# CMU-SAFARI/RawAlign

Measured on AMD Instinct MI355X. Metric: DTW GCUPS, higher is better.
Workload: dtype f32; 1 GPU; ecoli_k12_4.6Mb_r9.4_sparse_banded0.10; reads_per_gpu=16384, genome_bp=4600000, border_constraint=sparse, fill_method=banded=0.10, batches_in_flight=4

## Files before the change

rawalign_amd/csrc/rawdtw_runs.hip:

```cpp

#include "rawdtw_dp.h"

namespace rawdtw {

namespace {

constexpr int kT = 256;

__device__ __forceinline__ int d_slanted_radius(uint32_t n, uint32_t m, int r0)
{
    const uint32_t N = n > m ? n : m, M = n > m ? m : n;
    const uint32_t x = (N - M) * (uint32_t)r0 + N - 1u;
    uint32_t q;
    if (N < (1u << 11) && (uint32_t)r0 < (1u << 11)) {
        q = (uint32_t)((float)x * __builtin_amdgcn_rcpf((float)N));
        const int r = (int)x - (int)(q * N);
        q = r < 0 ? q - 1u : (r >= (int)N ? q + 1u : q);
    } else q = x / N;
    return r0 + (int)q;
}

__device__ uint32_t d_banded_cells(uint32_t n, uint32_t m, int R)
{
    const uint32_t N = n > m ? n : m, M = n > m ? m : n;
    const int P = R + ((R % 2 == 0) ? 1 : 0), S = R + ((R % 2 == 1) ? 1 : 0);
    uint32_t cells = 1;
    int row = 0;
    uint32_t rem = 0;
    for (uint32_t col = 1; col < N; col++) {
        rem += M;
        const bool adv = rem >= N;
        if (adv) { rem -= N; row++; }
        for (int pass = adv ? 0 : 1; pass < 2; pass++) {
            const int len = pass == 0 ? S : P;
            const int si = pass == 0 ? (int)col + S / 2 - 1 : (int)col + P / 2;
            const int sj = pass == 0 ? row - S / 2 : row - P / 2;
            int lo = 0, hi = len;
            lo = max(lo, si - (int)N + 1);
            lo = max(lo, -sj);
            hi = min(hi, si + 1);
            hi = min(hi, (int)M - sj);
            if (hi > lo) cells += (uint32_t)(hi - lo);
        }
    }
    return cells;
}

struct Part {
    uint32_t n, m;
    int R;
    bool asc;
    bool tile;
};

__device__ __forceinline__ Part classify(const StreamArgs &a, const rawdtw_anchor_t s, const rawdtw_anchor_t e)
{
    Part p;
    p.asc = e.target_position >= s.target_position && e.query_position >= s.query_position;
    p.m = e.target_position - s.target_position + 1;
    p.n = e.query_position - s.query_position + 1;
    int r0 = (int)((float)p.n * a.frac);
    r0 = r0 > 1 ? r0 : 1;
    const uint32_t N = p.n > p.m ? p.n : p.m, dr = (N - (p.n > p.m ? p.m : p.n)) * (uint32_t)r0;
    p.R = r0 + (dr > 0u ? 1 : 0) + (dr > N ? 1 : 0);
    p.tile = p.asc && p.n < 0x7fffffffu && p.m < 0x7fffffffu && N <= a.lane_max_n && r0 <= a.lane_max_radius &&
             dr <= (uint32_t)(a.lane_max_radius - r0) * N;
    return p;
}

__device__ __forceinline__ uint64_t find_chain(const uint64_t *__restrict__ anchor_off, uint64_t n_chains, uint64_t x, int lane)
{
    uint64_t lo = 0, hi = n_chains;
    while (hi - lo > 1) {
        const uint64_t step = (hi - lo + 63) / 64;
        const uint64_t p = lo + (uint64_t)lane * step;
        const bool le = p < hi && anchor_off[p] <= x;
        const int cnt = __popcll(__ballot(le));
        const uint64_t nlo = lo + (uint64_t)(cnt - 1) * step;
        hi = min(hi, nlo + step);
        lo = nlo;
    }
    return lo;
}

__device__ __forceinline__ void wave_lds_sync()
{
    __builtin_amdgcn_fence(__ATOMIC_RELEASE, "wavefront");
    __builtin_amdgcn_wave_barrier();
    __builtin_amdgcn_fence(__ATOMIC_ACQUIRE, "wavefront");
}

__device__ __forceinline__ uint32_t wave_scan_incl(uint32_t x)
{
    x += (uint32_t)__builtin_amdgcn_update_dpp(0, (int)x, 0x111, 0xf, 0xf, false);
    x += (uint32_t)__builtin_amdgcn_update_dpp(0, (int)x, 0x112, 0xf, 0xf, false);
    x += (uint32_t)__builtin_amdgcn_update_dpp(0, (int)x, 0x114, 0xf, 0xf, false);
    x += (uint32_t)__builtin_amdgcn_update_dpp(0, (int)x, 0x118, 0xf, 0xf, false);
    x += (uint32_t)__builtin_amdgcn_update_dpp(0, (int)x, 0x142, 0xa, 0xf, false);
    x += (uint32_t)__builtin_amdgcn_update_dpp(0, (int)x, 0x143, 0xc, 0xf, false);
    return x;
}

struct StepMap { uint32_t set, q, t; };
__device__ __forceinline__ StepMap compose(const StepMap later, const StepMap earlier)
{
    if (later.set) return later;
    return StepMap{earlier.set, earlier.set ? earlier.q - later.q : earlier.q + later.q, earlier.set ? earlier.t - later.t : earlier.t + later.t};
}
#define RAWDTW_DPP_MAP(m, ctrl, rowmask)                                                                                      \
    StepMap{(uint32_t)__builtin_amdgcn_update_dpp(0, (int)(m).set, ctrl, rowmask, 0xf, false),                                  \
            (uint32_t)__builtin_amdgcn_update_dpp(0, (int)(m).q, ctrl, rowmask, 0xf, false),                                    \
            (uint32_t)__builtin_amdgcn_update_dpp(0, (int)(m).t, ctrl, rowmask, 0xf, false)}
__device__ __forceinline__ StepMap wave_scan_maps(StepMap m)
{
    m = compose(m, RAWDTW_DPP_MAP(m, 0x111, 0xf));
    m = compose(m, RAWDTW_DPP_MAP(m, 0x112, 0xf));
    m = compose(m, RAWDTW_DPP_MAP(m, 0x114, 0xf));
    m = compose(m, RAWDTW_DPP_MAP(m, 0x118, 0xf));
    m = compose(m, RAWDTW_DPP_MAP(m, 0x142, 0xa));
    m = compose(m, RAWDTW_DPP_MAP(m, 0x143, 0xc));
    return m;
}

__device__ __forceinline__ bool mask_bit(const uint32_t *mask, uint32_t p) { return (mask[p >> 5] >> (p & 31u)) & 1u; }

template <int NT>
__device__ __forceinline__ bool mark_chain_starts(const StreamArgs &a, uint64_t c0, uint64_t base, uint32_t at, uint32_t *mask)
{
    bool ok = true;
    for (uint64_t c = c0 + threadIdx.x;; c += NT) {
        uint64_t s = ~0ull;
        if (c <= a.n_chains) {
            s = a.anchor_off[c];
            if (s >= base && s <= base + at) atomicOr(&mask[(uint32_t)(s - base) >> 5], 1u << ((uint32_t)(s - base) & 31u));
            if (c < a.n_chains && s < base + at && a.anchor_off[c + 1] == s) ok = false;
        }
        if (!__syncthreads_or(threadIdx.x == NT - 1 && c < a.n_chains && s < base + at)) break;
    }
    return ok;
}

}

__device__ __forceinline__ void chain_desc_body(const StreamArgs &a, ChainDesc *__restrict__ chains, const uint64_t c)
{
    if (c >= a.n_chains) return;
    const uint64_t a0 = a.anchor_off[c], a1 = a.anchor_off[c + 1];
    ChainDesc d;
    d.job_first = a1 >= 2 ? a1 - 2 : 0;
    d.n_jobs = a1 > a0 ? (uint32_t)(a1 - a0 - 1) : 0u;
    d.descending = 1; d.span = 0; d.num_aligned = 0;
    if (a1 > a0) {
        const rawdtw_anchor_t first = a.anchors[a1 - 1], last = a.anchors[a0];
        d.span = last.query_position - first.query_position + 1;
        d.num_aligned = (last.query_position - first.query_position) + d.n_jobs;
        if (d.n_jobs && ((uint64_t)a.read_base[c] + last.query_position + 1ull > a.n_ev || a.ref_base[c] + last.target_position + 1ull > a.n_ref))
            atomicMin(&a.cnt[kCntBad], (unsigned long long)a0);
    } else atomicAdd(&a.cnt[kCntUnsupported], 1ull);
    chains[c] = d;
}

template <int NT>
__device__ __forceinline__ void fold_order_body(const uint64_t n_chains, const uint64_t *__restrict__ anchor_off, uint32_t *__restrict__ order)
{
    constexpr uint32_t kBins = 1024, kB = kBins / NT;
    constexpr uint32_t kC = 4;
    __shared__ uint32_t hist[kBins];
    __shared__ uint32_t wsum[NT / 64];
    const uint32_t tid = threadIdx.x, lane = tid & 63u, wv = tid >> 6;
    auto bucket = [](uint64_t anchors) { return 1023u - (uint32_t)min<uint64_t>(anchors ? anchors - 1 : 0, 1023ull); };
    auto keys = [&](uint64_t c0, uint32_t (&b)[kC]) {
        uint64_t lo[kC], hi[kC];
#pragma unroll
        for (uint32_t q = 0; q < kC; q++) {
            const uint64_t c = min(c0 + (uint64_t)q * NT, n_chains - 1);
            lo[q] = anchor_off[c]; hi[q] = anchor_off[c + 1];
        }
#pragma unroll
        for (uint32_t q = 0; q < kC; q++) b[q] = bucket(hi[q] - lo[q]);
    };
    for (uint32_t i = tid; i < kBins; i += NT) hist[i] = 0;
    __syncthreads();
    for (uint64_t c0 = tid; c0 < n_chains; c0 += (uint64_t)NT * kC) {
        uint32_t b[kC];
        keys(c0, b);
#pragma unroll
        for (uint32_t q = 0; q < kC; q++)
            if (c0 + (uint64_t)q * NT < n_chains) atomicAdd(&hist[b[q]], 1u);
    }
    __syncthreads();
    uint32_t v[kB], mine = 0;
#pragma unroll
    for (uint32_t q = 0; q < kB; q++) { v[q] = hist[tid * kB + q]; mine += v[q]; }
    uint32_t incl = mine;
#pragma unroll
    for (int d = 1; d < 64; d <<= 1) {
        const uint32_t o = (uint32_t)__shfl_up((int)incl, d);
        if (lane >= (uint32_t)d) incl += o;
    }
    if (lane == 63) wsum[wv] = incl;
    __syncthreads();
    uint32_t at = incl - mine;
    for (uint32_t w = 0; w < wv; w++) at += wsum[w];
#pragma unroll
    for (uint32_t q = 0; q < kB; q++) { hist[tid * kB + q] = at; at += v[q]; }
    __syncthreads();
    for (uint64_t c0 = tid; c0 < n_chains; c0 += (uint64_t)NT * kC) {
        uint32_t b[kC];
        keys(c0, b);
#pragma unroll
        for (uint32_t q = 0; q < kC; q++)
            if (c0 + (uint64_t)q * NT < n_chains) order[atomicAdd(&hist[b[q]], 1u)] = (uint32_t)(c0 + (uint64_t)q * NT);
    }
}

struct RunTab {
    uint32_t lo[2][kStreamMaxSeg];
    uint32_t end[2][kStreamMaxSeg];
    int32_t D[2][kStreamMaxSeg];
    long long src[2][kStreamMaxSeg];
};

constexpr uint32_t kScanUnit = 8192, kScanKI = 8;
constexpr uint32_t kScanT = 512, kScanTC = 1024;
static_assert(kScanUnit == RAWDTW_COMPACT_STRIDE, "the compact hand-over is decoded unit by unit");
template <bool COMPACT>
__device__ __forceinline__ void scan_unit_body(const StreamArgs &a, const uint32_t unit)
{
    constexpr int NT = COMPACT ? (int)kScanTC : (int)kScanT, KI = (int)kScanKI;
    constexpr uint32_t AT = kScanUnit, kWords = AT / 32 + 1, kHalf = (uint32_t)NT * KI, kHalves = AT / kHalf;
    static_assert(kHalves * kHalf == AT && (!COMPACT || kHalves == 1), "a unit in whole passes; the compact form in one");
    __shared__ uint32_t s_mask[kWords], s_pre[kWords];
    __shared__ uint32_t s_ocnt, s_obase, s_cls[kStreamClasses];
    __shared__ unsigned long long s_stats[3];
    __shared__ uint64_t s_c0;
    __shared__ uint32_t s_todo;
    constexpr uint32_t kOList = 2048;
    __shared__ uint32_t s_olist[kOList];
    const int tid = threadIdx.x, lane = tid & 63;
    const uint64_t base = (uint64_t)unit * AT;
    for (uint32_t w = tid; w < kWords; w += NT) s_mask[w] = 0;
    if (tid == 0) { s_ocnt = 0; s_todo = 0; }
    if (tid < 3) s_stats[tid] = 0;
    if (tid < (int)kStreamClasses) s_cls[tid] = 0;
    const uint64_t i0 = base + (uint64_t)tid * KI;
    rawdtw_anchor_t an[KI + 1];
    uint4 steps8 = make_uint4(0u, 0u, 0u, 0u);
    if (COMPACT) { if (i0 < a.n_anchors) steps8 = *reinterpret_cast<const uint4 *>(a.steps + i0); }
    else {
#pragma unroll
        for (int k = 0; k <= KI; k++) an[k] = i0 + k < a.n_anchors ? a.anchors[i0 + k] : rawdtw_anchor_t{0, 0};
    }
    const rawdtw_anchor_t *const anchors_rd = COMPACT ? a.anchors_w : a.anchors;
    if (tid < 64) {
        const uint64_t c = find_chain(a.anchor_off, a.n_chains, base, lane);
        if (tid == 0) s_c0 = c;
    }
    __syncthreads();
    const uint64_t c0 = s_c0;
    if (!mark_chain_starts<NT>(a, c0, base, AT, s_mask)) atomicAdd(&a.cnt[kCntUnsupported], 1ull);
    {
        static_assert(kWords <= (uint32_t)NT, "one mask word a thread");
        __shared__ uint32_t s_wsum[NT / 64];
        const uint32_t pc = (uint32_t)tid < kWords ? __popc(s_mask[tid]) : 0u;
        uint32_t incl = pc;
#pragma unroll
        for (int d = 1; d < 64; d <<= 1) {
            const uint32_t o = (uint32_t)__shfl_up((int)incl, d);
            if (lane >= d) incl += o;
        }
        if (lane == 63) s_wsum[tid >> 6] = incl;
        __syncthreads();
        uint32_t pre = 0;
        for (int w = 0; w < (tid >> 6); w++) pre += s_wsum[w];
        if ((uint32_t)tid < kWords) s_pre[tid] = pre + incl - pc;
    }
    __syncthreads();
    auto chain_at = [&](uint32_t p) {
        return c0 + (s_pre[p >> 5] + __popc(s_mask[p >> 5] & (0xffffffffu >> (31u - (p & 31u)))) - (s_mask[0] & 1u));
    };
    if (COMPACT) {
        static_assert(KI == 8, "eight 2-byte steps a thread");
        __shared__ StepMap s_wagg[NT / 64];
        __shared__ uint2 s_first[NT];
        const uint32_t sv[8] = {steps8.x & 0xffffu, steps8.x >> 16, steps8.y & 0xffffu, steps8.y >> 16,
                                steps8.z & 0xffffu, steps8.z >> 16, steps8.w & 0xffffu, steps8.w >> 16};
        StepMap part[KI];
        StepMap run{0u, 0u, 0u};
#pragma unroll
        for (int k = 0; k < KI; k++) {
            const uint32_t p = (uint32_t)tid * KI + k;
            const uint64_t i = base + p;
            StepMap m{0u, 0u, 0u};
            if (i < a.n_anchors) {
                if (mask_bit(s_mask, p)) { const rawdtw_anchor_t h = a.heads[chain_at(p)]; m = StepMap{1u, h.query_position, h.target_position}; }
                else if (p == 0) { const rawdtw_anchor_t h = a.unit_abs[unit]; m = StepMap{1u, h.query_position, h.target_position}; }
                else if (sv[k] == 0xffffu) {
                    uint64_t lo = 0, hi = a.n_wide;
                    while (lo < hi) { const uint64_t mid = (lo + hi) >> 1; if (a.wide[mid].index < (uint32_t)i) lo = mid + 1; else hi = mid; }
                    if (lo < a.n_wide && a.wide[lo].index == (uint32_t)i) m = StepMap{0u, a.wide[lo].query_step, a.wide[lo].target_step};
                    else atomicMin(&a.cnt[kCntBad], (unsigned long long)i);
                } else m = StepMap{0u, sv[k] & 0xffu, sv[k] >> 8};
            }
            run = compose(m, run);
            part[k] = run;
        }
        const StepMap incl = wave_scan_maps(run);
        if (lane == 63) s_wagg[tid >> 6] = incl;
        __syncthreads();
        StepMap pre = RAWDTW_DPP_MAP(incl, 0x138, 0xf);
        {
            StepMap wpre{0u, 0u, 0u};
            for (int w = 0; w < (tid >> 6); w++) wpre = compose(s_wagg[w], wpre);
            pre = compose(pre, wpre);
        }
#pragma unroll
        for (int k = 0; k < KI; k++) {
            const StepMap f = compose(part[k], pre);
            an[k] = rawdtw_anchor_t{f.t, f.q};
            if (i0 + k < a.n_anchors) a.anchors_w[i0 + k] = an[k];
        }
        s_first[tid] = make_uint2(an[0].target_position, an[0].query_position);
        __syncthreads();
        if (tid + 1 < NT) { const uint2 x = s_first[tid + 1]; an[KI] = rawdtw_anchor_t{x.x, x.y}; }
        else an[KI] = base + AT < a.n_anchors ? a.unit_abs[unit + 1] : rawdtw_anchor_t{0, 0};
    }

    uint32_t my_tiles = 0, my_bytes = 0;
    unsigned long long my_obytes = 0;
    uint32_t o_rec[kHalves][KI];
#pragma unroll
    for (uint32_t h = 0; h < kHalves; h++) {
    const uint64_t ih = i0 + (uint64_t)h * kHalf;
    if (h) {
#pragma unroll
        for (int k = 0; k <= KI; k++) an[k] = ih + k < a.n_anchors ? a.anchors[ih + k] : rawdtw_anchor_t{0, 0};
    }
    uint32_t half_tiles = 0;
#pragma unroll
    for (int k = 0; k < KI; k++) {
        o_rec[h][k] = 0xffffffffu;
        const uint32_t p = h * kHalf + (uint32_t)tid * KI + k;
        const uint64_t i = base + p;
        if (i >= a.n_anchors || mask_bit(s_mask, p + 1)) continue;
        const Part pt = classify(a, an[k + 1], an[k]);
        if (!pt.asc || pt.n >= 0x7fffffffu || pt.m >= 0x7fffffffu) { atomicMin(&a.cnt[kCntBad], (unsigned long long)i); continue; }
        if (pt.tile) { my_tiles++; half_tiles++; my_bytes += 4u * (pt.n + pt.m) + 36u; continue; }
        int r0 = (int)((float)pt.n * a.frac);
        r0 = r0 > 1 ? r0 : 1;
        const int R = d_slanted_radius(pt.n, pt.m, r0);
        const uint32_t N = pt.n > pt.m ? pt.n : pt.m, K = (uint32_t)R + 1u;
        uint32_t cls;
        if (R >= 1 && R <= a.side_lane_radius && N <= a.lane_max_n) cls = kClsL0 + side_lane_bucket(N);
        else if (K <= 8) cls = kClsM0 + side_lane_bucket(N);
        else if (K <= 16) cls = kClsG16;
        else if (K <= 256) cls = N >= 1024 ? kClsW0 : N >= 256 ? kClsW0 + 1 : N >= 64 ? kClsW0 + 2 : kClsW0 + 3;
        else { atomicAdd(&a.cnt[kCntUnsupported], 1ull); continue; }
        my_obytes += 4ull * ((unsigned long long)pt.n + pt.m) + 36ull;
        {
            const uint32_t slot = atomicAdd(&s_ocnt, 1u);
            if (slot < kOList) s_olist[slot] = p | (cls << 13) | ((uint32_t)R << 18);
            else o_rec[h][k] = slot | (cls << 16) | ((uint32_t)R << 21);
        }
        atomicAdd(&s_cls[cls], 1u);
    }
    {
        const unsigned long long any_tile = __ballot(half_tiles != 0u);
        if (lane == 0 && any_tile) atomicOr(&s_todo, 1u << ((h * kHalf + (uint32_t)tid * KI) / a.tile_anchors));
    }
    }
    {
        unsigned long long packed = (unsigned long long)my_tiles | ((unsigned long long)my_bytes << 20);
        for (int off = 32; off > 0; off >>= 1) packed += __shfl_down(packed, off);
        if (lane == 0) { atomicAdd(&s_stats[0], packed & 0xfffffull); atomicAdd(&s_stats[1], packed >> 20); }
        if (my_obytes) atomicAdd(&s_stats[2], my_obytes);
    }
    __syncthreads();
    if (tid == 0 && s_ocnt) s_obase = (uint32_t)atomicAdd(&a.cnt[kCntOthers], (unsigned long long)s_ocnt);
    if (tid == 0 && s_todo) {
        const uint32_t tiles_per_unit = AT / a.tile_anchors, todo = s_todo;
        uint64_t at = atomicAdd(&a.cnt[kCntTodo], (unsigned long long)__popc(todo));
        for (uint32_t t = 0; t < tiles_per_unit; t++)
            if ((todo >> t) & 1u) a.tlist[at++] = make_uint2(unit * tiles_per_unit + t, (uint32_t)chain_at(t * a.tile_anchors));
    }
    if (tid < 3) a.tile_stats[3ull * unit + tid] = s_stats[tid];
    if (tid < (int)kStreamClasses && s_cls[tid]) atomicAdd(&a.cnt[kCntCls0 + tid], (unsigned long long)s_cls[tid]);
    __syncthreads();
    auto side_record = [&](const uint32_t p, const uint32_t cls, const uint32_t R, const uint64_t q) {
        if (q >= a.others_cap) return;
        const uint64_t c = chain_at(p);
        const rawdtw_anchor_t e = anchors_rd[base + p];
        const rawdtw_anchor_t s = (COMPACT && p + 1u == AT) ? a.unit_abs[unit + 1] : anchors_rd[base + p + 1];
        DevJob d;
        d.ref_off = a.ref_base[c] + s.target_position;
        d.read_off = a.read_base[c] + s.query_position;
        d.n = e.query_position - s.query_position + 1;
        d.m = e.target_position - s.target_position + 1;
        d.R = (int32_t)R;
        d.flags = mask_bit(s_mask, p) ? 0u : kFlagExcludeLast;
        d.aux = (uint32_t)(base + p);
        a.omix[q] = d; a.ocls[q] = (uint8_t)cls;
    };
    for (uint32_t t = (uint32_t)tid; t < min(s_ocnt, kOList); t += NT) {
        const uint32_t w = s_olist[t];
        side_record(w & 0x1fffu, (w >> 13) & 0x1fu, w >> 18, (uint64_t)s_obase + t);
    }
    if (s_ocnt > kOList) {
        const uint64_t obase = s_obase;
#pragma unroll
        for (uint32_t h = 0; h < kHalves; h++)
#pragma unroll
            for (int k = 0; k < KI; k++) {
                if (o_rec[h][k] == 0xffffffffu) continue;
                side_record(h * kHalf + (uint32_t)tid * KI + k, (o_rec[h][k] >> 16) & 0x1fu, o_rec[h][k] >> 21, obase + (o_rec[h][k] & 0xffffu));
            }
    }
}

__device__ __forceinline__ void chain_desc_carry(const StreamArgs &a, ChainDesc *__restrict__ chains, const uint64_t c)
{
    if (c >= a.n_chains) return;
    const uint64_t f0 = a.full_off[c], f1 = a.full_off[c + 1], r0 = a.anchor_off[c], r1 = a.anchor_off[c + 1];
    const rawdtw_carry_t rec = a.carry[c];
    ChainDesc d;
    d.job_first = f1 >= 2 ? f1 - 2 : 0;
    d.n_jobs = f1 > f0 ? (uint32_t)(f1 - f0 - 1) : 0u;
    d.descending = 1; d.span = 0; d.num_aligned = 0;
    const bool counts_ok = (r1 - r0) + rec.parts == f1 - f0 && (rec.parts == 0 || (rec.prev_src != ~0ull && rec.prev_src + rec.parts <= a.prev_n_full));
    if (f1 > f0 && r1 > r0 && counts_ok) {
        const rawdtw_anchor_t last = a.anchors[r0], first = rec.parts ? rec.start : a.anchors[r1 - 1];
        d.span = last.query_position - first.query_position + 1;
        d.num_aligned = (last.query_position - first.query_position) + d.n_jobs;
        if (d.n_jobs && ((uint64_t)a.read_base[c] + last.query_position + 1ull > a.n_ev || a.ref_base[c] + last.target_position + 1ull > a.n_ref ||
                         first.query_position > last.query_position || first.target_position > last.target_position))
            atomicMin(&a.cnt[kCntBad], (unsigned long long)r0);
    } else if (f1 > f0) atomicMin(&a.cnt[kCntBad], (unsigned long long)r0);
    else atomicAdd(&a.cnt[kCntUnsupported], 1ull);
    chains[c] = d;
}

constexpr int kGatherT = 256;
__global__ __launch_bounds__(kGatherT) void k_gather(const StreamArgs a)
{
    const int lane = threadIdx.x & 63;
    const uint64_t c = (uint64_t)blockIdx.x * (kGatherT / 64) + (threadIdx.x >> 6);
    if (c >= a.n_chains) return;
    if (a.cnt[kCntBad] != ~0ull || a.cnt[kCntOverflow] != ~0ull || a.cnt[kCntUnsupported] != 0ull || a.cnt[kCntOthers] > a.others_cap) return;
    const uint64_t f0 = a.full_off[c], r0 = a.anchor_off[c], r1 = a.anchor_off[c + 1];
    const rawdtw_carry_t rec = a.carry[c];
    const uint64_t L = rec.parts, n_new = r1 > r0 ? r1 - r0 - 1 : 0;
    for (uint64_t k = (uint64_t)lane; k < n_new; k += 64) a.out_full[f0 + k] = a.out[r0 + k];
    if (!L) return;
    const bool prev_ok = a.prev_cnt[kCntBad] == ~0ull && a.prev_cnt[kCntUnsupported] == 0ull && a.prev_cnt[kCntOthers] <= a.prev_others_cap &&
                         a.prev_cnt[kCntOverflow] == ~0ull;
    if (!prev_ok) { if (lane == 0) atomicMin(&a.cnt[kCntBad], (unsigned long long)r0); return; }
    const float *src = a.prev_out_full + rec.prev_src;
    float *dst = a.out_full + f0 + n_new;
    for (uint64_t k = (uint64_t)lane; k < L; k += 64) {
        float cost = src[k];
        if (k == 0 && (rec.flags & 1u)) {
            const rawdtw_anchor_t e = a.anchors[r1 - 1];
            cost = cost - dist(a.ev[(uint64_t)a.read_base[c] + e.query_position], a.ref[a.ref_base[c] + e.target_position]);
        }
        dst[k] = cost;
    }
}

__global__ __launch_bounds__(kScanT, 8) void k_scan(const StreamArgs a, ChainDesc *__restrict__ chains, uint32_t *__restrict__ order)
{
    const uint32_t b = blockIdx.x, n_desc = (uint32_t)((a.n_chains + kScanT - 1) / kScanT);
    if (b == 0) { if (a.n_chains && order) fold_order_body<(int)kScanT>(a.n_chains, a.carry ? a.full_off : a.anchor_off, order); }
    else if (b <= n_desc) {
        if (a.carry) chain_desc_carry(a, chains, (uint64_t)(b - 1) * kScanT + threadIdx.x);
        else chain_desc_body(a, chains, (uint64_t)(b - 1) * kScanT + threadIdx.x);
    }
    else scan_unit_body<false>(a, b - 1 - n_desc);
}

__global__ __launch_bounds__(kScanTC) void k_scan_compact(const StreamArgs a, uint32_t *__restrict__ order)
{
    const uint32_t b = blockIdx.x;
    if (b == 0) { if (a.n_chains && order) fold_order_body<(int)kScanTC>(a.n_chains, a.anchor_off, order); }
    else scan_unit_body<true>(a, b - 1);
}
__global__ __launch_bounds__(kScanT) void k_scan_desc(const StreamArgs a, ChainDesc *__restrict__ chains)
{
    chain_desc_body(a, chains, (uint64_t)blockIdx.x * kScanT + threadIdx.x);
}

constexpr int kPlanT = 256;
__global__ __launch_bounds__(kPlanT, 3) void k_plan(const StreamArgs a)
{
    constexpr int KI = 8;
    constexpr uint32_t kWords = kStreamTile / 32 + 1;
    static_assert(kStreamTile == 64 * KI, "a wave a tile, eight items a lane");
    __shared__ uint32_t s_hist[kPlanT / 64][kSortBins];
    __shared__ RunTab s_rtab[kPlanT / 64];
    __shared__ uint32_t s_tmp[kPlanT / 64][8];
    __shared__ uint32_t s_maskw[kPlanT / 64][kWords + 1], s_prew[kPlanT / 64][kWords + 1];
    const int tid = threadIdx.x, lane = tid & 63;
    const uint32_t wv = (uint32_t)tid >> 6;
    const uint32_t li = blockIdx.x * (kPlanT / 64) + wv;
    const uint2 te = a.tlist[min(li, a.n_tiles - 1u)];
    if (a.cnt[kCntBad] != ~0ull || a.cnt[kCntUnsupported] != 0ull || a.cnt[kCntOthers] > a.others_cap) return;
    const uint32_t n_list = (uint32_t)min<unsigned long long>(a.cnt[kCntTodo], (unsigned long long)a.n_tiles);
    if (li >= n_list) return;
    const uint32_t tile = te.x;
    const uint64_t c0 = te.y, base = (uint64_t)tile * kStreamTile;
    uint32_t *hist = s_hist[wv], *tmp = s_tmp[wv], *mask = s_maskw[wv], *pre = s_prew[wv];
    RunTab &rt = s_rtab[wv];
    rawdtw_anchor_t an[KI + 1];
    const uint64_t i0 = base + (uint64_t)lane * KI;
#pragma unroll
    for (int k = 0; k <= KI; k++) an[k] = i0 + k < a.n_anchors ? a.anchors[i0 + k] : rawdtw_anchor_t{0, 0};
    if ((uint32_t)lane < kWords) mask[lane] = 0;
    wave_lds_sync();
    for (uint64_t c = c0 + (uint32_t)lane;; c += 64) {
        const bool in = c <= a.n_chains;
        const uint64_t st = in ? a.anchor_off[c] : ~0ull;
        if (in && st >= base && st <= base + kStreamTile) atomicOr(&mask[(uint32_t)(st - base) >> 5], 1u << ((uint32_t)(st - base) & 31u));
        const unsigned long long more = __ballot(in && st < base + kStreamTile);
        if (!(more >> 63)) break;
    }
    wave_lds_sync();
    {
        const uint32_t pc = (uint32_t)lane < kWords ? __popc(mask[lane]) : 0u;
        const uint32_t incl = wave_scan_incl(pc);
        if ((uint32_t)lane < kWords) pre[lane] = incl - pc;
    }
    wave_lds_sync();
    auto chain_at = [&](uint32_t p) { return c0 + (pre[p >> 5] + __popc(mask[p >> 5] & (0xffffffffu >> (31u - (p & 31u)))) - (mask[0] & 1u)); };
    uint32_t tm[KI];
#pragma unroll
    for (int k = 0; k < KI; k++) {
        const uint32_t p = (uint32_t)lane * KI + k;
        tm[k] = 0u;
        if (base + p >= a.n_anchors || mask_bit(mask, p + 1)) continue;
        const Part pt = classify(a, an[k + 1], an[k]);
        if (!pt.tile) continue;
        const uint32_t N = pt.n > pt.m ? pt.n : pt.m, M = pt.n > pt.m ? pt.m : pt.n;
        tm[k] = rec_shape(N, M, (uint32_t)pt.R, mask_bit(mask, p) ? 0u : 1u) | ((pt.n < pt.m ? 1u : 0u) << kItemSwapped) | (1u << kItemTile);
    }
    {
        const int t_first = (int)((tm[0] >> kItemTile) & 1u), t_last = (int)((tm[KI - 1] >> kItemTile) & 1u);
        const bool below = __builtin_amdgcn_update_dpp(0, t_last, 0x138, 0xf, 0xf, false) != 0;
        const bool above = __builtin_amdgcn_update_dpp(0, t_first, 0x130, 0xf, 0xf, false) != 0;
        auto contrib = [](const uint32_t t, uint32_t &c_r, uint32_t &c_f) {
            const bool tl = (t >> kItemTile) & 1u, starts = (t >> kItemRunStart) & 1u, ends = (t >> kItemRunEnd) & 1u, swap = (t >> kItemSwapped) & 1u;
            const uint32_t N = rec_n(t), M = rec_m(t), n = swap ? M : N, m = swap ? N : M;
            c_r = tl ? ((starts ? n + 3u : n - 1u) + (ends ? 3u : 0u)) | ((starts ? 1u : 0u) << kSumRunShift) : 0u;
            c_f = tl ? (starts ? m + 3u : m - 1u) + (ends ? 3u : 0u) : 0u;
        };
        uint32_t lr = 0, lf = 0;
#pragma unroll
        for (int k = 0; k < KI; k++) {
            const bool t = (tm[k] >> kItemTile) & 1u;
            const bool pred = k + 1 < KI ? ((tm[k + 1 < KI ? k + 1 : k] >> kItemTile) & 1u) != 0u : above;
            const bool succ = k > 0 ? ((tm[k > 0 ? k - 1 : 0] >> kItemTile) & 1u) != 0u : below;
            tm[k] |= ((t && !pred ? 1u : 0u) << kItemRunStart) | ((t && !succ ? 1u : 0u) << kItemRunEnd);
            uint32_t c_r, c_f;
            contrib(tm[k], c_r, c_f);
            lr += c_r; lf += c_f;
        }
        const uint32_t ir = wave_scan_incl(lr), jf = wave_scan_incl(lf);
        const uint32_t tot_r = (uint32_t)__builtin_amdgcn_readlane((int)ir, 63), tot_f = (uint32_t)__builtin_amdgcn_readlane((int)jf, 63);
        const uint32_t base_r = tot_r - (ir - lr), base_f = tot_f - (jf - lf);
        const uint32_t budget = a.lds_floats & ~3u;
        uint32_t u0 = 0, b0r = 0, b0f = 0, b0s = 0;
        uint32_t rec_off = 0;
        for (bool first = true;; first = false) {
            const bool all_fit = ((((tot_r & kSumFloatsMask) - b0r + 7u) & ~3u) + ((tot_f - b0f + 7u) & ~3u) <= budget) && ((tot_r >> kSumRunShift) - b0s + 1u <= kStreamMaxSeg);
            uint32_t u1 = kStreamTile, e_r = tot_r & kSumFloatsMask, e_f = tot_f, e_s = tot_r >> kSumRunShift;
            bool cut_run = false;
            if (!all_fit || u0 != 0u) {
                uint32_t fits = 0;
                {
                    uint32_t xr = base_r, xf = base_f;
#pragma unroll
                    for (int k = 0; k < KI; k++) {
                        uint32_t c_r, c_f;
                        contrib(tm[k], c_r, c_f);
                        const uint32_t u = kStreamTile - 1u - ((uint32_t)lane * KI + k), sr = xr & kSumFloatsMask, ss = xr >> kSumRunShift;
                        if (u >= u0 && ((sr - b0r + 7u) & ~3u) + ((xf - b0f + 7u) & ~3u) <= budget && ss - b0s + 1u <= kStreamMaxSeg) fits++;
                        xr -= c_r; xf -= c_f;
                    }
                }
                fits = (uint32_t)__builtin_amdgcn_readlane((int)wave_scan_incl(fits), 63);
                u1 = min(u0 + fits, kStreamTile);
                if (u1 <= u0) { if (lane == 0) atomicMin(&a.cnt[kCntOverflow], (unsigned long long)tile); break; }
                {
                    uint32_t xr = base_r, xf = base_f;
#pragma unroll
                    for (int k = 0; k < KI; k++) {
                        uint32_t c_r, c_f;
                        contrib(tm[k], c_r, c_f);
                        const uint32_t u = kStreamTile - 1u - ((uint32_t)lane * KI + k);
                        if (u == u1 - 1u) { tmp[0] = xr & kSumFloatsMask; tmp[1] = xf; tmp[2] = xr >> kSumRunShift; }
                        if (u == u0) tmp[3] = ((tm[k] >> kItemTile) & 1u) && !((tm[k] >> kItemRunStart) & 1u) ? 1u : 0u;
                        xr -= c_r; xf -= c_f;
                    }
                }
                wave_lds_sync();
                e_r = tmp[0]; e_f = tmp[1]; e_s = tmp[2];
                cut_run = tmp[3] != 0u;
            }
            const uint32_t region = (e_r - b0r + (cut_run ? 4u : 0u) + 3u) & ~3u;
            const uint32_t n_runs = e_s - b0s + (cut_run ? 1u : 0u);
            const bool last = u1 >= kStreamTile;
            uint32_t slot = li;
            if (!first) {
                uint32_t sl = 0;
                if (lane == 0) sl = a.n_tiles + (uint32_t)atomicAdd(&a.cnt[kCntPool], 1ull);
                slot = (uint32_t)__builtin_amdgcn_readfirstlane((int)sl);
                if (slot >= a.n_slots) { if (lane == 0) atomicMin(&a.cnt[kCntOverflow], (unsigned long long)tile); break; }
            }
            for (uint32_t b = (uint32_t)lane; b < kSortBins; b += 64u) hist[b] = 0;
            wave_lds_sync();
            {
                uint32_t xr = base_r, xf = base_f;
#pragma unroll
                for (int k = 0; k < KI; k++) {
                    uint32_t c_r, c_f;
                    contrib(tm[k], c_r, c_f);
                    const uint32_t u = kStreamTile - 1u - ((uint32_t)lane * KI + k);
                    const uint32_t sr = xr & kSumFloatsMask, sf = xf, ss = xr >> kSumRunShift;
                    xr -= c_r; xf -= c_f;
                    if (!((tm[k] >> kItemTile) & 1u) || u < u0 || u >= u1) continue;
                    const uint32_t N = rec_n(tm[k]), R = rec_radius(tm[k]);
                    const bool starts = ((tm[k] >> kItemRunStart) & 1u) || u == u0, ends = ((tm[k] >> kItemRunEnd) & 1u) || u == u1 - 1u;
                    atomicAdd(&hist[sort_bin(R, N)], 1u);
                    const uint32_t adj = (cut_run && u > u0) ? 1u : 0u;
                    const uint32_t g = ss - b0s + (cut_run ? 1u : 0u) - 1u;
                    if (starts) {
                        const rawdtw_anchor_t sa = an[k + 1];
                        rt.lo[0][g] = sr - (c_r & kSumFloatsMask) - b0r + 4u * adj; rt.lo[1][g] = sf - c_f - b0f + 4u * adj;
                        rt.D[0][g] = (int32_t)sa.query_position; rt.D[1][g] = (int32_t)sa.target_position;
                        rt.src[0][g] = (long long)((uint32_t)lane * KI + k);
                    }
                    if (ends) { rt.end[0][g] = an[k].query_position + 1u; rt.end[1][g] = an[k].target_position + 1u; }
                }
            }
            wave_lds_sync();
            if ((uint32_t)lane < n_runs) {
                const uint32_t g = (uint32_t)lane;
                const uint32_t q_r = rt.lo[0][g], q_f = rt.lo[1][g], sq = (uint32_t)rt.D[0][g], st = (uint32_t)rt.D[1][g];
                const uint64_t c = chain_at((uint32_t)rt.src[0][g]);
                const uint64_t rb = a.ref_base[c];
                const uint32_t qb = a.read_base[c];
                const uint32_t off_r = qb + sq;
                const uint64_t off_f = rb + st;
                const uint32_t p_r = q_r + ((off_r - q_r) & 3u), p_f = region + q_f + (((uint32_t)off_f - q_f) & 3u);
                rt.lo[0][g] = p_r & ~3u; rt.lo[1][g] = p_f & ~3u;
                rt.D[0][g] = (int32_t)(p_r - sq); rt.D[1][g] = (int32_t)(p_f - st);
                rt.src[0][g] = (long long)off_r - (long long)p_r; rt.src[1][g] = (long long)off_f - (long long)p_f;
            }
            wave_lds_sync();
            const uint32_t h0 = hist[3 * lane], h1 = hist[3 * lane + 1], h2 = hist[3 * lane + 2];
            const uint32_t hsum = h0 + h1 + h2, hincl = wave_scan_incl(hsum);
            const uint32_t n_jobs = (uint32_t)__builtin_amdgcn_readlane((int)hincl, 63);
            hist[3 * lane] = hincl - hsum; hist[3 * lane + 1] = hincl - hsum + h0; hist[3 * lane + 2] = hincl - hsum + h0 + h1;
            static_assert(kSortBins == 3 * 64 && kSortBinRadius1 % 3 == 2, "three bins a lane; the first radius-1 bin is a lane's third");
            const uint32_t n_hi = (uint32_t)__builtin_amdgcn_readlane((int)(hincl - hsum + h0 + h1), kSortBinRadius1 / 3);
            wave_lds_sync();
            {
                uint32_t xs = base_r >> kSumRunShift;
#pragma unroll
                for (int k = 0; k < KI; k++) {
                    const uint32_t u = kStreamTile - 1u - ((uint32_t)lane * KI + k), ss = xs;
                    xs -= (tm[k] >> kItemRunStart) & (tm[k] >> kItemTile) & 1u;
                    if (!((tm[k] >> kItemTile) & 1u) || u < u0 || u >= u1) continue;
                    const uint32_t N = rec_n(tm[k]), R = rec_radius(tm[k]);
                    const uint32_t place = atomicAdd(&hist[sort_bin(R, N)], 1u);
                    const uint32_t g = ss - b0s + (cut_run ? 1u : 0u) - 1u;
                    const rawdtw_anchor_t sa = an[k + 1];
                    const uint32_t p_r = sa.query_position + (uint32_t)rt.D[0][g], p_f = sa.target_position + (uint32_t)rt.D[1][g];
                    const bool swap = (tm[k] >> kItemSwapped) & 1u;
                    a.recs[(uint64_t)tile * kStreamRecStride + rec_off + place] = make_uint2(rec_windows(swap ? p_f : p_r, swap ? p_r : p_f), rec_with_item(tm[k], u));
                }
            }
            if ((uint32_t)lane < 2u * n_runs) {
                const uint32_t g = (uint32_t)lane >> 1, w = (uint32_t)lane & 1u;
                const long long src = rt.src[w][g];
                a.runtab[(uint64_t)slot * (2u * kStreamMaxSeg) + lane] =
                    make_uint4(rt.lo[w][g] >> 2, (rt.end[w][g] + (uint32_t)rt.D[w][g] + 3u) >> 2, order_src_lo(src), order_src_hi(src));
            }
            wave_lds_sync();
            if (lane == 0) a.todo[slot] = make_uint4(tile, slot, pass_counts(n_jobs, n_runs, n_hi), pass_place(region, rec_off));
            if (last) break;
            rec_off += (n_jobs + 1u) & ~1u;
            if (rec_off + (kStreamTile - u1) > kStreamRecStride) { if (lane == 0) atomicMin(&a.cnt[kCntOverflow], (unsigned long long)tile); break; }
            u0 = u1; b0r = e_r; b0f = e_f; b0s = e_s;
        }
    }
}

constexpr uint32_t kSideGroups = 64;
__global__ __launch_bounds__(1024) void k_side(const StreamArgs a)
{
    constexpr int NT = 1024;
    const uint32_t group = blockIdx.x;
    const uint64_t n_other = min<uint64_t>(a.cnt[kCntOthers], a.others_cap);
    const uint64_t per = (n_other + kSideGroups - 1) / kSideGroups;
    const uint64_t lo = min(n_other, (uint64_t)group * per), hi = min(n_other, lo + per);
    if (lo >= hi) return;
    __shared__ uint32_t s_n[kStreamClasses];
    __shared__ uint64_t s_at[kStreamClasses];
    if (threadIdx.x < kStreamClasses) s_n[threadIdx.x] = 0;
    __syncthreads();
    for (uint64_t i = lo + threadIdx.x; i < hi; i += NT) atomicAdd(&s_n[a.ocls[i]], 1u);
    __syncthreads();
    if (threadIdx.x < kStreamClasses) {
        uint64_t base = 0;
        for (uint32_t c = 0; c < threadIdx.x; c++) base += a.cnt[kCntCls0 + c];
        const uint32_t mine = s_n[threadIdx.x];
        s_at[threadIdx.x] = base + (mine ? atomicAdd(&a.cnt[kCntCur0 + threadIdx.x], (unsigned long long)mine) : 0ull);
        s_n[threadIdx.x] = 0;
    }
    __syncthreads();
    for (uint64_t i = lo + threadIdx.x; i < hi; i += NT) {
        const uint32_t cls = a.ocls[i];
        const uint64_t pos = s_at[cls] + atomicAdd(&s_n[cls], 1u);
        if (pos < a.others_cap) a.ojobs[pos] = a.omix[i];
    }
}

namespace {

constexpr uint32_t kStamps = 10;

__device__ __forceinline__ uint32_t wave_max_u32(uint32_t n_max)
{
    n_max = max(n_max, (uint32_t)__builtin_amdgcn_update_dpp(0, (int)n_max, 0x111, 0xf, 0xf, false));
    n_max = max(n_max, (uint32_t)__builtin_amdgcn_update_dpp(0, (int)n_max, 0x112, 0xf, 0xf, false));
    n_max = max(n_max, (uint32_t)__builtin_amdgcn_update_dpp(0, (int)n_max, 0x114, 0xf, 0xf, false));
    n_max = max(n_max, (uint32_t)__builtin_amdgcn_update_dpp(0, (int)n_max, 0x118, 0xf, 0xf, false));
    n_max = max(n_max, (uint32_t)__builtin_amdgcn_update_dpp(0, (int)n_max, 0x142, 0xa, 0xf, false));
    n_max = max(n_max, (uint32_t)__builtin_amdgcn_update_dpp(0, (int)n_max, 0x143, 0xc, 0xf, false));
    return (uint32_t)__builtin_amdgcn_readlane((int)n_max, 63);
}

__device__ __forceinline__ float stream_lane_job(const float *LA, const float *LB, uint32_t N, uint32_t M, uint32_t R, bool excl, bool act)
{
    const unsigned long long r12 = __ballot(R <= 2u), r1 = __ballot(R == 1u), r2 = __ballot(R == 2u);
    const uint32_t n_max = wave_max_u32(N);
    float res;
    if (~r1 == 0ull) res = lane_dp_r1(LA, LB, N, n_max);
    else if (~r2 == 0ull) res = lane_dp_r2(LA, LB, N, M, n_max);
    else if (~r12 == 0ull) res = lane_dp_r12(LA, LB, N, M, R, n_max);
    else res = lane_dp_gen(LA, LB, N, M, R, n_max);
    if (act && excl) res = res - dist(LA[N - 1], LB[M - 1]);
    return res;
}

template <int SLOTS>
__device__ __forceinline__ void lane_global_wave(const DevJob *__restrict__ jobs, uint32_t count, uint32_t wave, int lane,
                                                 const float *__restrict__ ev, const float *__restrict__ ref, float *__restrict__ out)
{
    const uint32_t idx = wave * 64u + (uint32_t)lane;
    const bool have = idx < count;
    const DevJob jb = jobs[have ? idx : count - 1u];
    const float *A = ev + jb.read_off;
    const float *B = ref + jb.ref_off;
    uint32_t N = jb.n, M = jb.m;
    if (N < M) {
        const float *tp = A; A = B; B = tp;
        const uint32_t tn = N; N = M; M = tn;
    }
    uint32_t n_max = N;
#pragma unroll
    for (int d = 1; d < 64; d <<= 1) n_max = max(n_max, (uint32_t)__shfl_xor((int)n_max, d));
    n_max = (uint32_t)__builtin_amdgcn_readfirstlane((int)n_max);
    float res = SLOTS == 4 ? lane_dp_gen<true>(A, B, N, M, (uint32_t)jb.R, n_max) : lane_dp_k8(A, B, N, M, jb.R, n_max);
    if (have) {
        if (jb.flags & kFlagExcludeLast) res = res - dist(A[N - 1], B[M - 1]);
        out[jb.aux] = res;
    }
}

__device__ __forceinline__ uint32_t next_tile(const StreamArgs &a, const uint32_t dbg, uint32_t &head, uint32_t n_tiles, const uint32_t base = 0u)
{
    if (dbg & 8u) {
        const uint32_t t = head;
        head += gridDim.x;
        return t < n_tiles ? t : 0xffffffffu;
    }
    for (uint32_t tries = 0; tries < 8; tries++) {
        const uint32_t h = (head + tries) & 7u;
        const uint32_t k = (uint32_t)atomicAdd(&a.cnt[kCntHeads + 16 * h], 1ull);
        const uint64_t t = (uint64_t)base + (uint64_t)k * 8u + h;
        if (t < n_tiles) { head = h; return (uint32_t)t; }
    }
    return 0xffffffffu;
}


}

__global__ __launch_bounds__(256) void k_wide(const StreamArgs a)
{
    const uint32_t dbg = a.debug;
    constexpr uint32_t kWaves = 4;
    __shared__ __attribute__((aligned(16))) float s_w[kWaves][kWbandLdsFloats];
    __shared__ uint32_t s_next;
    const int tid = threadIdx.x, lane = tid & 63;
    const uint32_t wv = (uint32_t)tid >> 6;
    if (a.cnt[kCntBad] != ~0ull || a.cnt[kCntUnsupported] != 0ull || a.cnt[kCntOthers] > a.others_cap) return;
    if (!(dbg & 4u)) {
        uint64_t n_w = 0;
#pragma unroll
        for (uint32_t c = kClsW0; c < kClsW0 + 4; c++) n_w += a.cnt[kCntCls0 + c];
        const uint64_t n_g16 = a.cnt[kCntCls0 + kClsG16];
        uint64_t n_l = 0, n_m = 0;
#pragma unroll
        for (uint32_t c = kClsL0; c < kClsL0 + kClsLCount; c++) n_l += a.cnt[kCntCls0 + c];
#pragma unroll
        for (uint32_t c = kClsM0; c < kClsM0 + kClsMCount; c++) n_m += a.cnt[kCntCls0 + c];
        const uint64_t it_g16 = (n_g16 + 3) / 4, it_l = (n_l + 63) / 64, it_m = (n_m + 63) / 64, items = n_w + it_g16 + it_l + it_m;
        const uint32_t G = gridDim.x;
        const uint32_t n_items = (uint32_t)min<uint64_t>(items, 0xffffffffull);
        if (tid == 0) s_next = 0;
        __syncthreads();
        for (;;) {
            uint32_t kq = 0;
            if (lane == 0) kq = atomicAdd(&s_next, 1u);
            kq = (uint32_t)__builtin_amdgcn_readfirstlane((int)kq);
            const uint64_t first = (uint64_t)kq * G;
            if (first >= n_items) break;
            const uint64_t it = first + ((kq & 1u) ? G - 1u - blockIdx.x : blockIdx.x);
            if (it >= n_items) continue;
            if (it < n_w) {
                if (dbg & 32u) continue;
                const DevJob jb = a.ojobs[it];
                const uint32_t len = max(jb.n, jb.m);
                if (len >= 256u) __builtin_amdgcn_s_setprio(3);
                else if (len >= 96u) __builtin_amdgcn_s_setprio(2);
                else __builtin_amdgcn_s_setprio(1);
                wreg_small_job(jb, lane, a.ev, a.ref, a.out, s_w[wv]);
                __builtin_amdgcn_s_setprio(0);
            }
            else if (dbg & 64u) continue;
            else if (it < n_w + it_g16) grp_wave<16>(a.ojobs + n_w, (uint32_t)n_g16, (uint32_t)(it - n_w), lane, a.ev, a.ref, a.out);
            else if (it < n_w + it_g16 + it_l) lane_global_wave<4>(a.ojobs + n_w + n_g16, (uint32_t)n_l, (uint32_t)(it - n_w - it_g16), lane, a.ev, a.ref, a.out);
            else lane_global_wave<8>(a.ojobs + n_w + n_g16 + n_l, (uint32_t)n_m, (uint32_t)(it - n_w - it_g16 - it_l), lane, a.ev, a.ref, a.out);
        }
    }

}

template <int TT, bool DIAG>
__global__ __launch_bounds__(TT, 4) void k_runs(const StreamArgs a, const uint32_t lds_floats)
{
    const uint32_t dbg = DIAG ? a.debug : 0u;
    constexpr uint32_t kWaves = TT / 64, kRT = 2u * kStreamMaxSeg;
    extern __shared__ __attribute__((aligned(16))) float smem[];
    float *win = smem;
    uint2 *rec = reinterpret_cast<uint2 *>(smem + lds_floats);
    uint4 *rtab = reinterpret_cast<uint4 *>(rec + kStreamTile);
    __shared__ uint4 s_ent[2];
    __shared__ uint32_t s_seq;
    const int tid = threadIdx.x, lane = tid & 63;
    const uint32_t wv = (uint32_t)tid >> 6;

    if (a.cnt[kCntBad] != ~0ull || a.cnt[kCntOverflow] != ~0ull || a.cnt[kCntUnsupported] != 0ull || a.cnt[kCntOthers] > a.others_cap) return;

    auto dma16 = [](const void *src, void *dst) {
        __builtin_amdgcn_global_load_lds((const __attribute__((address_space(1))) void *)src, (__attribute__((address_space(3))) void *)dst, 16, 0, 0);
    };
    auto fetch_recs = [&](const uint4 e) {
        const uint32_t n_jobs = pass_jobs(e.z), pieces = (n_jobs + 1u) >> 1;
        const uint2 *src = a.recs + (uint64_t)e.x * kStreamRecStride + pass_rec0(e.w);
        for (uint32_t q0 = wv * 64u; q0 < pieces; q0 += (uint32_t)TT)
            if (q0 + (uint32_t)lane < pieces) dma16(src + 2u * (q0 + (uint32_t)lane), rec + 2u * q0);
    };
    auto fetch_orders = [&](const uint4 e, const uint32_t buf) {
        const uint32_t n_ord = 2u * pass_runs(e.z);
        if ((uint32_t)lane < n_ord) dma16(a.runtab + (uint64_t)e.y * kRT + lane, rtab + buf * kRT);
    };

    __shared__ unsigned long long s_stamp[kWaves][kStamps];
    unsigned long long t_prev = 0;
    const bool stamps = DIAG && (dbg & 256u) != 0u;
    if (stamps) {
        if (lane < (int)kStamps) s_stamp[wv][lane] = 0;
        t_prev = __builtin_amdgcn_s_memtime();
    }
    auto stamp = [&](const int ph) {
        if (!stamps) return;
        const unsigned long long t = __builtin_amdgcn_s_memtime();
        if (lane == 0) s_stamp[wv][ph] += t - t_prev;
        t_prev = t;
    };
    const uint32_t n_first = (uint32_t)min<unsigned long long>(a.cnt[kCntTodo], (unsigned long long)a.n_tiles);
    const uint32_t n_pass = n_first + (uint32_t)min<unsigned long long>(a.cnt[kCntPool], (unsigned long long)(a.n_slots - a.n_tiles));
    auto entry_of = [&](const uint32_t i) { return a.todo[i < n_first ? i : a.n_tiles + (i - n_first)]; };
    uint32_t head = (dbg & 8u) ? blockIdx.x : (blockIdx.x & 7u);
    const uint32_t q_base = (dbg & 8u) ? 0u : 2u * gridDim.x;
    unsigned long long ticket = 0;
    bool more = false;
    const uint4 none = make_uint4(0xffffffffu, 0u, 0u, 0u);
    uint4 e_next = none, e_load = none;
    if (wv == 0) {
        uint32_t i0 = 0xffffffffu, i1 = 0xffffffffu;
        if (dbg & 8u) {
            if (tid == 0) {
                i0 = next_tile(a, dbg, head, n_pass);
                i1 = i0 != 0xffffffffu ? next_tile(a, dbg, head, n_pass) : 0xffffffffu;
                more = i1 != 0xffffffffu;
            }
        } else {
            i0 = blockIdx.x < n_pass ? blockIdx.x : 0xffffffffu;
            i1 = blockIdx.x + gridDim.x < n_pass ? blockIdx.x + gridDim.x : 0xffffffffu;
            if (tid == 0) {
                more = i1 != 0xffffffffu;
                if (more) ticket = atomicAdd(&a.cnt[kCntHeads + 16 * head], 1ull);
            }
        }
        i0 = (uint32_t)__builtin_amdgcn_readfirstlane((int)i0);
        i1 = (uint32_t)__builtin_amdgcn_readfirstlane((int)i1);
        const uint4 e0 = i0 != 0xffffffffu ? entry_of(i0) : none;
        if (i1 != 0xffffffffu) e_next = entry_of(i1);
        if (tid == 0) s_ent[0] = e0;
    }
    __syncthreads();
    if (s_ent[0].x == 0xffffffffu) return;
    if (wv == kWaves - 1u) fetch_orders(s_ent[0], 0u);
    __builtin_amdgcn_s_waitcnt(0x0f70);
    __syncthreads();
    auto run_dp = [&](const uint2 *rc_base, const uint32_t n_jobs, const uint32_t n_hi_e, const uint32_t end_nom) {
        uint32_t n3;
        {
            const uint32_t R0 = rec_radius(rc_base[min((uint32_t)lane, n_jobs - 1u)].y);
            n3 = (uint32_t)__popcll(__ballot((uint32_t)lane < n_jobs && R0 == 3u));
        }
        const uint32_t n_hi = min(max(n_hi_e, n3), n_jobs);
        const uint32_t n_chunks = chunk_map_count(n3, n_hi, n_jobs);
        for (uint32_t c = wv; !(dbg & 1u);) {
            if (c >= n_chunks) break;
            if ((dbg & 512u) && c == 0u) { uint32_t cn0 = 0; if (lane == 0) cn0 = atomicAdd(&s_seq, 1u); c = (uint32_t)__builtin_amdgcn_readfirstlane((int)cn0); continue; }
            if ((dbg & 1024u) && c != 0u) break;
            const ChunkRange cr = chunk_map_range(n3, n_hi, n_jobs, c);
            if (cr.quad) {
                const uint32_t r = cr.first + ((uint32_t)lane >> 2);
                const bool act = r < cr.end;
                const uint2 rc = rc_base[act ? r : cr.end - 1u];
                const uint32_t N = rec_n(rc.y), M = rec_m(rc.y), u = rec_item(rc.y);
                const float *LA = win + rec_long(rc.x), *LB = win + rec_short(rc.x);
                float res = quad_dp_r3(LA, LB, N, M, lane, wave_max_u32(N));
                if (act && ((lane & 3) == 2)) {
                    if (rec_excl(rc.y)) res = res - dist(LA[N - 1], LB[M - 1]);
                    a.out[end_nom - 1u - u] = res;
                }
// ... 375 lines not shown
```

Before: 883.3 GCUPS.

## Search chain index with whole workgroup and cache chain bases in LDS

The chain lookup at the start of each scan unit now uses every thread of the workgroup instead of a single wave. Each round probes NT points, which cuts the number of dependent global-load rounds. In the tile kernel, the ref_base and read_base values of the first 64 chains are loaded during the mask pass and kept in LDS, so the later per-run lookups can skip dependent global loads. Tile and chain indices are made wave-uniform via readfirstlane. The cost is extra barriers per search round, extra LDS in RunTab, and an up-front load that some tiles may not need.

Result: no change. 889.2 GCUPS (median of 6 runs) (+0.7%).

```diff
diff --git a/rawalign_amd/csrc/rawdtw_find_chain.h b/rawalign_amd/csrc/rawdtw_find_chain.h
--- /dev/null
+++ b/rawalign_amd/csrc/rawdtw_find_chain.h
@@ -0,0 +1,28 @@
+#pragma once
+#include <stdint.h>
+
+#if defined(__HIPCC__) || defined(__CUDACC__)
+#define RAWDTW_FIND_FN __host__ __device__ inline
+#else
+#define RAWDTW_FIND_FN inline
+#endif
+
+namespace rawdtw {
+
+struct ChainRange {
+    uint64_t lo, hi;
+};
+
+RAWDTW_FIND_FN ChainRange find_chain_begin(uint64_t n_chains) { return ChainRange{0, n_chains}; }
+RAWDTW_FIND_FN bool find_chain_done(const ChainRange r) { return r.hi - r.lo <= 1; }
+template <uint32_t P>
+RAWDTW_FIND_FN uint64_t find_chain_step(const ChainRange r) { return (r.hi - r.lo + (P - 1u)) / P; }
+RAWDTW_FIND_FN uint64_t find_chain_probe(const ChainRange r, uint64_t step, uint32_t i) { return r.lo + (uint64_t)i * step; }
+RAWDTW_FIND_FN bool find_chain_probe_in(const ChainRange r, uint64_t probe) { return probe < r.hi; }
+RAWDTW_FIND_FN ChainRange find_chain_narrow(const ChainRange r, uint64_t step, int n_le)
+{
+    const uint64_t lo = r.lo + (uint64_t)(n_le - 1) * step;
+    return ChainRange{lo, r.hi < lo + step ? r.hi : lo + step};
+}
+
+}
diff --git a/rawalign_amd/csrc/rawdtw_runs.hip b/rawalign_amd/csrc/rawdtw_runs.hip
--- a/rawalign_amd/csrc/rawdtw_runs.hip
+++ b/rawalign_amd/csrc/rawdtw_runs.hip
@@ -1,5 +1,6 @@
 
 #include "rawdtw_dp.h"
+#include "rawdtw_find_chain.h"
 
 namespace rawdtw {
 
@@ -70,17 +71,36 @@
 
 __device__ __forceinline__ uint64_t find_chain(const uint64_t *__restrict__ anchor_off, uint64_t n_chains, uint64_t x, int lane)
 {
-    uint64_t lo = 0, hi = n_chains;
-    while (hi - lo > 1) {
-        const uint64_t step = (hi - lo + 63) / 64;
-        const uint64_t p = lo + (uint64_t)lane * step;
-        const bool le = p < hi && anchor_off[p] <= x;
+    ChainRange r = find_chain_begin(n_chains);
+    while (!find_chain_done(r)) {
+        const uint64_t step = find_chain_step<64>(r);
+        const uint64_t p = find_chain_probe(r, step, (uint32_t)lane);
+        const bool le = find_chain_probe_in(r, p) && anchor_off[p] <= x;
         const int cnt = __popcll(__ballot(le));
-        const uint64_t nlo = lo + (uint64_t)(cnt - 1) * step;
-        hi = min(hi, nlo + step);
-        lo = nlo;
-    }
-    return lo;
+        r = find_chain_narrow(r, step, cnt);
+    }
+    return r.lo;
+}
+
+template <int NT>
+__device__ __forceinline__ uint64_t find_chain_wg(const uint64_t *__restrict__ anchor_off, uint64_t n_chains, uint64_t x, uint32_t (*cnt)[NT / 64])
+{
+    const uint32_t tid = threadIdx.x;
+    ChainRange r = find_chain_begin(n_chains);
+    for (uint32_t round = 0; !find_chain_done(r); round ^= 1u) {
+        const uint64_t step = find_chain_step<(uint32_t)NT>(r);
+        const uint64_t p = find_chain_probe(r, step, tid);
+        const bool le = find_chain_probe_in(r, p) && anchor_off[p] <= x;
+        const unsigned long long b = __ballot(le);
+        if ((tid & 63u) == 0u) cnt[round][tid >> 6] = (uint32_t)__popcll(b);
+        __syncthreads();
+        uint32_t n_le = 0;
+#pragma unroll
+        for (int w = 0; w < NT / 64; w++) n_le += cnt[round][w];
+        n_le = (uint32_t)__builtin_amdgcn_readfirstlane((int)n_le);
+        r = find_chain_narrow(r, step, (int)max(n_le, 1u));
+    }
+    return r.lo;
 }
 
 __device__ __forceinline__ void wave_lds_sync()
@@ -219,6 +239,8 @@
     uint32_t end[2][kStreamMaxSeg];
     int32_t D[2][kStreamMaxSeg];
     long long src[2][kStreamMaxSeg];
+    uint64_t chain_f[64];
+    uint32_t chain_r[64];
 };
 
 constexpr uint32_t kScanUnit = 8192, kScanKI = 8;
@@ -233,7 +255,7 @@
     __shared__ uint32_t s_mask[kWords], s_pre[kWords];
     __shared__ uint32_t s_ocnt, s_obase, s_cls[kStreamClasses];
     __shared__ unsigned long long s_stats[3];
-    __shared__ uint64_t s_c0;
+    __shared__ uint32_t s_find[2][NT / 64];
     __shared__ uint32_t s_todo;
     constexpr uint32_t kOList = 2048;
     __shared__ uint32_t s_olist[kOList];
@@ -252,12 +274,8 @@
         for (int k = 0; k <= KI; k++) an[k] = i0 + k < a.n_anchors ? a.anchors[i0 + k] : rawdtw_anchor_t{0, 0};
     }
     const rawdtw_anchor_t *const anchors_rd = COMPACT ? a.anchors_w : a.anchors;
-    if (tid < 64) {
-        const uint64_t c = find_chain(a.anchor_off, a.n_chains, base, lane);
-        if (tid == 0) s_c0 = c;
-    }
-    __syncthreads();
-    const uint64_t c0 = s_c0;
+    const uint64_t c0 = find_chain_wg<NT>(a.anchor_off, a.n_chains, base, s_find);
+    __syncthreads();
     if (!mark_chain_starts<NT>(a, c0, base, AT, s_mask)) atomicAdd(&a.cnt[kCntUnsupported], 1ull);
     {
         static_assert(kWords <= (uint32_t)NT, "one mask word a thread");
@@ -377,7 +395,7 @@
     }
     __syncthreads();
     if (tid == 0 && s_ocnt) s_obase = (uint32_t)atomicAdd(&a.cnt[kCntOthers], (unsigned long long)s_ocnt);
-    if (tid == 0 && s_todo) {
+    if (tid == 64 && s_todo) {
         const uint32_t tiles_per_unit = AT / a.tile_anchors, todo = s_todo;
         uint64_t at = atomicAdd(&a.cnt[kCntTodo], (unsigned long long)__popc(todo));
         for (uint32_t t = 0; t < tiles_per_unit; t++)
@@ -505,8 +523,8 @@
     if (a.cnt[kCntBad] != ~0ull || a.cnt[kCntUnsupported] != 0ull || a.cnt[kCntOthers] > a.others_cap) return;
     const uint32_t n_list = (uint32_t)min<unsigned long long>(a.cnt[kCntTodo], (unsigned long long)a.n_tiles);
     if (li >= n_list) return;
-    const uint32_t tile = te.x;
-    const uint64_t c0 = te.y, base = (uint64_t)tile * kStreamTile;
+    const uint32_t tile = (uint32_t)__builtin_amdgcn_readfirstlane((int)te.x);
+    const uint64_t c0 = (uint32_t)__builtin_amdgcn_readfirstlane((int)te.y), base = (uint64_t)tile * kStreamTile;
     uint32_t *hist = s_hist[wv], *tmp = s_tmp[wv], *mask = s_maskw[wv], *pre = s_prew[wv];
     RunTab &rt = s_rtab[wv];
     rawdtw_anchor_t an[KI + 1];
@@ -515,9 +533,14 @@
     for (int k = 0; k <= KI; k++) an[k] = i0 + k < a.n_anchors ? a.anchors[i0 + k] : rawdtw_anchor_t{0, 0};
     if ((uint32_t)lane < kWords) mask[lane] = 0;
     wave_lds_sync();
-    for (uint64_t c = c0 + (uint32_t)lane;; c += 64) {
+    bool first_round = true;
+    for (uint64_t c = c0 + (uint32_t)lane;; c += 64, first_round = false) {
         const bool in = c <= a.n_chains;
         const uint64_t st = in ? a.anchor_off[c] : ~0ull;
+        if (first_round) {
+            const uint64_t cb = min(c, a.n_chains - 1u);
+            rt.chain_f[lane] = a.ref_base[cb]; rt.chain_r[lane] = a.read_base[cb];
+        }
         if (in && st >= base && st <= base + kStreamTile) atomicOr(&mask[(uint32_t)(st - base) >> 5], 1u << ((uint32_t)(st - base) & 31u));
         const unsigned long long more = __ballot(in && st < base + kStreamTile);
         if (!(more >> 63)) break;
@@ -645,8 +668,9 @@
                 const uint32_t g = (uint32_t)lane;
                 const uint32_t q_r = rt.lo[0][g], q_f = rt.lo[1][g], sq = (uint32_t)rt.D[0][g], st = (uint32_t)rt.D[1][g];
                 const uint64_t c = chain_at((uint32_t)rt.src[0][g]);
-                const uint64_t rb = a.ref_base[c];
-                const uint32_t qb = a.read_base[c];
+                const bool parked = c - c0 < 64u;
+                const uint64_t rb = parked ? rt.chain_f[c - c0] : a.ref_base[c];
+                const uint32_t qb = parked ? rt.chain_r[c - c0] : a.read_base[c];
                 const uint32_t off_r = qb + sq;
                 const uint64_t off_f = rb + st;
                 const uint32_t p_r = q_r + ((off_r - q_r) & 3u), p_f = region + q_f + (((uint32_t)off_f - q_f) & 3u);
```
